# 10XGenomics/rust-pseudoaligner

Measured on AMD Instinct MI355X. Metric: reads/sec pseudoaligned (whole node) on synthetic 150bp reads, higher is better.
Workload: dtype u64; 1 GPU; config3: ~202k-transcript synthetic GENCODE-scale index (K=24), error-free 150bp reads; read_len=150, k=24, transcripts=201914, kmers=103866252, index_bytes=7185579820

## Files before the change

### rust-pseudoaligner_amd/csrc/count_sort.hip

```cpp
#include <hip/hip_runtime.h>

#include <algorithm>

#include "kernels.hpp"
#include "pa_common.hpp"

namespace pa {
namespace {

constexpr uint32_t NO_KEY = 0xFFFFFFFFu;
#ifndef PA_MAX_BINS
#define PA_MAX_BINS 256
#endif
constexpr uint32_t MAX_BINS = PA_MAX_BINS;
constexpr uint64_t PA_COUNT_DIRECT_MAX_READS = 1u << 16;
constexpr uint32_t BIN_SLOTS = 1u << PA_KEY_BIN_SHIFT;
constexpr uint32_t CS_BLOCK = 1024;

struct KeyTops {
    const unsigned long long* top;
    uint64_t cap;
    const unsigned long long* extra_top;
    uint64_t extra_cap;
};
__device__ __forceinline__ uint64_t stream_len(const KeyTops k, uint64_t unused = 0) {
    (void)unused;
    unsigned long long t = *k.top, x = k.extra_top ? *k.extra_top : 0ull;
    if (t > k.cap) t = k.cap;
    if (x > k.extra_cap) x = k.extra_cap;
    return t + x;
}

constexpr uint32_t PT_BLOCK = 512, PT_PER = 16, PT_TILE = PT_BLOCK * PT_PER;

__device__ __forceinline__ uint64_t main_len(const KeyTops k) { const unsigned long long t = *k.top; return t < k.cap ? t : k.cap; }
__device__ __forceinline__ uint64_t extra_len(const KeyTops k) {
    const unsigned long long x = k.extra_top ? *k.extra_top : 0ull;
    return x < k.extra_cap ? x : k.extra_cap;
}
__device__ __forceinline__ uint32_t tiles_of(uint64_t n) { return (uint32_t)((n + PT_TILE - 1) / PT_TILE); }

__global__ __launch_bounds__(PT_BLOCK) void pa_keys_part_kernel(const uint32_t* __restrict__ keys, const KeyTops keys_top, uint32_t pass, uint32_t nbins,
                                                                uint32_t tcap, uint16_t* __restrict__ sorted, uint32_t* __restrict__ run_off) {
    __shared__ uint32_t cnt[MAX_BINS], lbase[MAX_BINS + 1];
    __shared__ __attribute__((aligned(16))) uint16_t stage[PT_TILE];
    const uint64_t m = main_len(keys_top);
    const uint64_t seg0 = pass ? m : 0, len = pass ? extra_len(keys_top) : m;
    const uint32_t tile0 = pass ? tiles_of(m) : 0u, ntiles = tiles_of(len);
    for (uint32_t t = blockIdx.x; t < ntiles; t += gridDim.x) {
        for (uint32_t b = threadIdx.x; b < nbins; b += PT_BLOCK) cnt[b] = 0;
        __syncthreads();
        const uint64_t t0 = (uint64_t)t * PT_TILE;
        uint32_t k[PT_PER], pos[PT_PER];
        const uint4* src = reinterpret_cast<const uint4*>(keys + seg0 + t0) + threadIdx.x;
#pragma unroll
        for (uint32_t j = 0; j < PT_PER / 4; ++j) {
            const uint64_t i = t0 + 4ull * (j * PT_BLOCK + threadIdx.x);
            const uint4 v = i < len ? src[j * PT_BLOCK] : uint4{NO_KEY, NO_KEY, NO_KEY, NO_KEY};
            k[4 * j] = v.x; k[4 * j + 1] = v.y; k[4 * j + 2] = v.z; k[4 * j + 3] = v.w;
        }
#pragma unroll
        for (uint32_t j = 0; j < PT_PER; ++j) pos[j] = k[j] != NO_KEY ? atomicAdd(&cnt[k[j] >> PA_KEY_BIN_SHIFT], 1u) : 0u;
        __syncthreads();
        for (uint32_t b = threadIdx.x; b <= nbins; b += PT_BLOCK) {
            uint32_t s = 0;
            for (uint32_t j = 0; j < b; ++j) s += cnt[j];
            lbase[b] = s;
            run_off[(uint64_t)b * tcap + tile0 + t] = s;
        }
        __syncthreads();
#pragma unroll
        for (uint32_t j = 0; j < PT_PER; ++j)
            if (k[j] != NO_KEY) stage[lbase[k[j] >> PA_KEY_BIN_SHIFT] + pos[j]] = (uint16_t)(k[j] & (BIN_SLOTS - 1));
        __syncthreads();
        uint4* dst = reinterpret_cast<uint4*>(sorted + (uint64_t)(tile0 + t) * PT_TILE);
        const uint32_t n8 = (lbase[nbins] + 7) / 8;
        for (uint32_t i = threadIdx.x; i < n8; i += PT_BLOCK) dst[i] = reinterpret_cast<const uint4*>(stage)[i];
        __syncthreads();
    }
}

constexpr uint32_t CG_LANES = 16, CG_DEPTH = 8;
__global__ __launch_bounds__(CS_BLOCK) void pa_keys_count_kernel(const uint16_t* __restrict__ src, const uint32_t* __restrict__ run_off, uint32_t tcap,
                                                                 const KeyTops keys_top, uint32_t parts, unsigned long long* __restrict__ counts,
                                                                 uint64_t counts_len) {
    extern __shared__ uint32_t tab[];
    const uint32_t bin = blockIdx.x / parts, part = blockIdx.x % parts;
    const uint64_t slot0 = (uint64_t)bin << PA_KEY_BIN_SHIFT;
    const uint32_t nslots = (uint32_t)(counts_len - slot0 < BIN_SLOTS ? counts_len - slot0 : BIN_SLOTS);
    for (uint32_t i = threadIdx.x; i < nslots; i += CS_BLOCK) tab[i] = 0;
    __syncthreads();
    const uint32_t ntiles = tiles_of(main_len(keys_top)) + tiles_of(extra_len(keys_top));
    const uint32_t ta = (uint32_t)((uint64_t)ntiles * part / parts), tb = (uint32_t)((uint64_t)ntiles * (part + 1) / parts);
    const uint32_t gl = threadIdx.x % CG_LANES, group = threadIdx.x / CG_LANES;
    const uint4* q = reinterpret_cast<const uint4*>(src);
    for (uint32_t t = ta + group; t < tb; t += CS_BLOCK / CG_LANES) {
        const uint64_t base = (uint64_t)t * PT_TILE;
        const uint64_t a = base + run_off[(uint64_t)bin * tcap + t], b = base + run_off[(uint64_t)(bin + 1) * tcap + t];
        const uint64_t a8 = (a + 7) & ~7ull, b8 = b & ~7ull;
        if (a8 >= b8) {
            for (uint64_t i = a + gl; i < b; i += CG_LANES) atomicAdd(&tab[src[i]], 1u);
            continue;
        }
        const uint32_t head = a + gl < a8 ? src[a + gl] : 0xFFFFu, tail = b8 + gl < b ? src[b8 + gl] : 0xFFFFu;
        for (uint64_t o0 = a8 / 8; o0 < b8 / 8; o0 += (uint64_t)CG_DEPTH * CG_LANES) {
            uint4 v[CG_DEPTH];
            bool in[CG_DEPTH];
#pragma unroll
            for (uint32_t j = 0; j < CG_DEPTH; ++j) {
                const uint64_t o = o0 + (uint64_t)j * CG_LANES + gl;
                in[j] = o < b8 / 8;
                v[j] = in[j] ? q[o] : uint4{0u, 0u, 0u, 0u};
            }
#pragma unroll
            for (uint32_t j = 0; j < CG_DEPTH; ++j)
                if (in[j]) {
                    atomicAdd(&tab[v[j].x & 0xFFFFu], 1u); atomicAdd(&tab[v[j].x >> 16], 1u);
                    atomicAdd(&tab[v[j].y & 0xFFFFu], 1u); atomicAdd(&tab[v[j].y >> 16], 1u);
                    atomicAdd(&tab[v[j].z & 0xFFFFu], 1u); atomicAdd(&tab[v[j].z >> 16], 1u);
                    atomicAdd(&tab[v[j].w & 0xFFFFu], 1u); atomicAdd(&tab[v[j].w >> 16], 1u);
                }
        }
        if (head != 0xFFFFu) atomicAdd(&tab[head], 1u);
        if (tail != 0xFFFFu) atomicAdd(&tab[tail], 1u);
    }
    __syncthreads();
    for (uint32_t i = threadIdx.x; i < nslots; i += CS_BLOCK) {
        const uint32_t c = tab[i];
        if (c) atomicAdd(counts + slot0 + i, (unsigned long long)c);
    }
}

__global__ __launch_bounds__(CS_BLOCK) void pa_keys_count_raw_kernel(const uint32_t* __restrict__ src, const KeyTops keys_top, unsigned long long* __restrict__ counts,
                                                                     uint64_t counts_len) {
    extern __shared__ uint32_t tab[];
    for (uint32_t i = threadIdx.x; i < counts_len; i += CS_BLOCK) tab[i] = 0;
    __syncthreads();
    const uint64_t n4 = stream_len(keys_top) / 4;
    const uint64_t a = n4 * blockIdx.x / gridDim.x, b = n4 * (blockIdx.x + 1) / gridDim.x;
    const uint4* q = reinterpret_cast<const uint4*>(src);
    for (uint64_t i = a + threadIdx.x; i < b; i += CS_BLOCK) {
        const uint4 v = q[i];
        if (v.x != NO_KEY) atomicAdd(&tab[v.x], 1u);
        if (v.y != NO_KEY) atomicAdd(&tab[v.y], 1u);
        if (v.z != NO_KEY) atomicAdd(&tab[v.z], 1u);
        if (v.w != NO_KEY) atomicAdd(&tab[v.w], 1u);
    }
    __syncthreads();
    for (uint32_t i = threadIdx.x; i < counts_len; i += CS_BLOCK) {
        const uint32_t c = tab[i];
        if (c) atomicAdd(counts + i, (unsigned long long)c);
    }
}

__global__ __launch_bounds__(256) void pa_keys_count_direct_kernel(const uint32_t* __restrict__ keys, const KeyTops keys_top, unsigned long long* __restrict__ counts) {
    const uint64_t n = stream_len(keys_top);
    for (uint64_t i = (uint64_t)blockIdx.x * blockDim.x + threadIdx.x; i < n; i += (uint64_t)gridDim.x * blockDim.x) {
        const uint32_t k = keys[i];
        if (k != NO_KEY) atomicAdd(counts + k, 1ull);
    }
}


}
uint64_t key_stream_capacity(uint64_t n_reads, uint32_t nwaves) {
    return (n_reads / PA_KEY_CHUNK + nwaves + 2) * PA_KEY_CHUNK;
}

static uint64_t nbins_of(uint64_t counts_len) { return (counts_len + BIN_SLOTS - 1) >> PA_KEY_BIN_SHIFT; }

static bool count_direct(uint64_t nbins, uint64_t n_reads) { return nbins > MAX_BINS || (nbins > 1 && n_reads <= PA_COUNT_DIRECT_MAX_READS); }

bool count_keys_partitioned(uint64_t counts_len, uint64_t n_reads) {
    const uint64_t nbins = nbins_of(counts_len);
    return nbins > 1 && !count_direct(nbins, n_reads);
}

static uint32_t tile_capacity(uint64_t keys_cap, uint64_t extra_cap) {
    return (uint32_t)((keys_cap + PT_TILE - 1) / PT_TILE + (extra_cap + PT_TILE - 1) / PT_TILE);
}

void count_keys_scratch(uint64_t counts_len, uint64_t n_reads, uint64_t keys_cap, uint64_t extra_cap, size_t* sorted_bytes, size_t* ctl_bytes) {
    *sorted_bytes = *ctl_bytes = 0;
    if (!count_keys_partitioned(counts_len, n_reads)) return;
    const uint64_t tcap = tile_capacity(keys_cap, extra_cap);
    *sorted_bytes = tcap * PT_TILE * sizeof(uint16_t);
    *ctl_bytes = (nbins_of(counts_len) + 1) * tcap * sizeof(uint32_t);
}

int launch_count_keys(const uint32_t* keys, const unsigned long long* keys_top_ptr, uint64_t keys_cap, const unsigned long long* extra_top, uint64_t extra_cap,
                      uint32_t* sorted, uint32_t* ctl, unsigned long long* counts, uint64_t counts_len, int num_cus, hipStream_t stream, uint64_t n_reads,
                      uint32_t pass) {
    if (counts_len == 0) return 0;
    const KeyTops keys_top{keys_top_ptr, keys_cap, extra_top, extra_cap};
    const uint64_t nbins = nbins_of(counts_len);
    const uint32_t cus = num_cus > 0 ? (uint32_t)num_cus : 256u;
    const bool partitioned = count_keys_partitioned(counts_len, n_reads);
    if (pass == 0) {
        if (!partitioned) return 0;
        const uint32_t tcap = tile_capacity(keys_cap, extra_cap);
        const uint32_t G = std::max<uint32_t>(1u, std::min<uint32_t>(cus * 4, (uint32_t)((keys_cap + PT_TILE - 1) / PT_TILE)));
        hipLaunchKernelGGL(pa_keys_part_kernel, dim3(G), dim3(PT_BLOCK), 0, stream, keys, keys_top, 0u, (uint32_t)nbins, tcap, reinterpret_cast<uint16_t*>(sorted), ctl);
        return (int)hipGetLastError();
    }
    const size_t lds = (size_t)(counts_len < BIN_SLOTS ? counts_len : BIN_SLOTS) * 4;
    if (lds > 48 * 1024) {
        hipError_t e = hipFuncSetAttribute(reinterpret_cast<const void*>(&pa_keys_count_kernel), hipFuncAttributeMaxDynamicSharedMemorySize, (int)lds);
        if (e == hipSuccess) e = hipFuncSetAttribute(reinterpret_cast<const void*>(&pa_keys_count_raw_kernel), hipFuncAttributeMaxDynamicSharedMemorySize, (int)lds);
        if (e != hipSuccess) return (int)e;
    }
    if (count_direct(nbins, n_reads)) {
        const uint32_t blocks = (uint32_t)std::min<uint64_t>((uint64_t)cus * 8, (keys_cap + extra_cap + 255) / 256 + 1);
        hipLaunchKernelGGL(pa_keys_count_direct_kernel, dim3(blocks), dim3(256), 0, stream, keys, keys_top, counts);
        return (int)hipGetLastError();
    }
    if (nbins == 1) {
        hipLaunchKernelGGL(pa_keys_count_raw_kernel, dim3(cus), dim3(CS_BLOCK), lds, stream, keys, keys_top, counts, counts_len);
        return (int)hipGetLastError();
    }
    const uint32_t tcap = tile_capacity(keys_cap, extra_cap);
    const uint32_t G1 = std::max<uint32_t>(1u, std::min<uint32_t>(cus * 4, (uint32_t)((extra_cap + PT_TILE - 1) / PT_TILE)));
    hipLaunchKernelGGL(pa_keys_part_kernel, dim3(G1), dim3(PT_BLOCK), 0, stream, keys, keys_top, 1u, (uint32_t)nbins, tcap, reinterpret_cast<uint16_t*>(sorted), ctl);
    uint32_t parts = std::max<uint32_t>(1u, (uint32_t)(cus / nbins));
    parts = std::max<uint32_t>(1u, (uint32_t)knob_int("PA_COUNT_PARTS", (int)parts));
    hipLaunchKernelGGL(pa_keys_count_kernel, dim3((uint32_t)nbins * parts), dim3(CS_BLOCK), lds, stream, reinterpret_cast<const uint16_t*>(sorted), (const uint32_t*)ctl, tcap,
                       keys_top, parts, counts, counts_len);
    return (int)hipGetLastError();
}

}
```

### rust-pseudoaligner_amd/csrc/resolve.hip

```cpp
#include <hip/hip_runtime.h>

#include "kernel_utils.hpp"
#include "kernels.hpp"
#include "lane_steps.hpp"

namespace pa {
namespace {

constexpr uint32_t NO_KEY = 0xFFFFFFFFu;
typedef uint32_t u32x4 __attribute__((ext_vector_type(4)));

constexpr uint32_t RV_PER = 4;

__global__ __launch_bounds__(256) void pa_resolve_kernel(const MapParams p, uint64_t defer_cap, uint64_t keys_cap) {
    __shared__ unsigned long long s_novel;
    if (threadIdx.x == 0) s_novel = 0;
    __syncthreads();
    const unsigned long long top = *p.defer_top;
    const uint64_t n = top < defer_cap ? top : defer_cap;
    const uint32_t lane = lane_id();
    const bool counting = p.keys != nullptr;
    uint32_t* keys_b = nullptr;
    if (counting) { const unsigned long long kt = *p.keys_top; keys_b = p.keys + (kt < keys_cap ? kt : keys_cap); }
    unsigned long long a_cur = 0, a_end = 0;
    uint32_t my_novel = 0;
    const uint64_t wave0 = ((uint64_t)blockIdx.x * blockDim.x + threadIdx.x) & ~63ull, nwave_lanes = (uint64_t)gridDim.x * blockDim.x;
    for (uint64_t i0 = wave0 * RV_PER; i0 < n; i0 += nwave_lanes * RV_PER) {
        u32x4 e0[RV_PER], e1[RV_PER];
        bool in[RV_PER], live[RV_PER];
        uint64_t idx[RV_PER];
#pragma unroll
        for (uint32_t j = 0; j < RV_PER; ++j) {
            idx[j] = i0 + 64ull * j + lane;
            in[j] = idx[j] < n;
            e0[j] = in[j] ? reinterpret_cast<const u32x4*>(p.defer)[2 * idx[j]] : u32x4{NO_KEY, 0u, 0u, 0u};
        }
#pragma unroll
        for (uint32_t j = 0; j < RV_PER; ++j) {
            live[j] = e0[j].x != NO_KEY;
            e1[j] = live[j] ? reinterpret_cast<const u32x4*>(p.defer)[2 * idx[j] + 1] : u32x4{0u, 0u, 0u, 0u};
        }
        uint32_t colour[RV_PER], want[RV_PER];
        uint32_t wsum = 0;
#pragma unroll
        for (uint32_t j = 0; j < RV_PER; ++j) {
            colour[j] = NO_CLASS;
            const uint32_t count = e0[j].w & 0x3FFFFFFFu;
            if (live[j] && (e0[j].w & PA_DEFER_WINDOW)) {
                uint32_t b1 = e1[j].x, m1 = e1[j].y, b2 = e1[j].z, m2 = e1[j].w;
                window_canon(b1, m1, b2, m2);
                colour[j] = window_class(p.ix, b1, m1, b2, m2);
            } else if (live[j]) {
                colour[j] = class_of_list(p.arena + e1[j].x, count, p.ix, p.class_table, p.class_table_size);
            }
            want[j] = (live[j] && (e0[j].w & PA_DEFER_WINDOW) && colour[j] == NO_CLASS) ? count : 0u;
            wsum += want[j];
        }
        const uint32_t incl = wave_incl_scan(wsum);
        const uint32_t total = (uint32_t)__builtin_amdgcn_readlane((int)incl, 63);
        if (total && a_cur + total > a_end) {
            const unsigned long long take = total > PA_ARENA_CHUNK ? total : PA_ARENA_CHUNK;
            unsigned long long base = 0;
            if (lane == 0) base = atomicAdd(p.arena_top, take);
            a_cur = ((unsigned long long)(uint32_t)__builtin_amdgcn_readfirstlane((int)(base >> 32)) << 32) | (uint32_t)__builtin_amdgcn_readfirstlane((int)base);
            a_end = a_cur + take;
        }
        unsigned long long my_off = a_cur + (incl - wsum);
        a_cur += total;
#pragma unroll
        for (uint32_t j = 0; j < RV_PER; ++j) {
            const uint32_t rid = e0[j].x, cov = e0[j].y, mm = e0[j].z, count = e0[j].w & 0x3FFFFFFFu;
            const bool window = live[j] && (e0[j].w & PA_DEFER_WINDOW);
            bool listed = live[j] && colour[j] == NO_CLASS;
            uint32_t arena_off = e1[j].x;
            if (window) {
                uint32_t class_off = PA_CLASS_REF | colour[j];
                if (want[j]) {
                    class_off = (uint32_t)my_off;
                    arena_off = (uint32_t)my_off;
                    if (my_off + count > p.arena_cap) { atomicOr(p.status, PA_STATUS_ARENA_FULL); listed = false; }
                    else {
                        uint32_t* dst = p.arena + my_off;
                        uint32_t k = 0;
                        for (uint32_t t = e1[j].y; t; t &= t - 1) dst[k++] = e1[j].x + (uint32_t)(__ffs((int)t) - 1);
                        for (uint32_t t = e1[j].w; t; t &= t - 1) dst[k++] = e1[j].z + (uint32_t)(__ffs((int)t) - 1);
                    }
                    my_off += count;
                }
                reinterpret_cast<u32x4*>(p.results)[rid] = u32x4{cov, mm | PA_MAPPED_BIT, class_off, count};
            }
            if (live[j] && p.colour_out) p.colour_out[rid] = colour[j];
            if (live[j] && colour[j] == NO_CLASS) ++my_novel;
            if (counting && in[j]) keys_b[idx[j]] = (live[j] && colour[j] != NO_CLASS) ? colour[j] : NO_KEY;
            if (p.novel_list) {
                const uint64_t m = __ballot(listed);
                if (m) {
                    const uint32_t first = (uint32_t)(__ffsll((unsigned long long)m) - 1);
                    unsigned long long nb = 0;
                    if (lane == first) nb = atomicAdd(p.novel_ctr, (unsigned long long)__popcll(m));
                    nb = ((unsigned long long)(uint32_t)__builtin_amdgcn_readlane((int)(nb >> 32), (int)first) << 32) | (uint32_t)__builtin_amdgcn_readlane((int)nb, (int)first);
                    if (listed) {
                        const unsigned long long at = nb + __builtin_amdgcn_mbcnt_hi((uint32_t)(m >> 32), __builtin_amdgcn_mbcnt_lo((uint32_t)m, 0u));
                        if (at < p.novel_cap) {
                            p.novel_list[2 * at] = arena_off;
                            p.novel_list[2 * at + 1] = count;
                        } else atomicOr(p.novel_status, PA_NOVEL_LIST_FULL);
                    }
                }
            }
        }
    }
    if (counting) {
        if (my_novel) atomicAdd(&s_novel, (unsigned long long)my_novel);
        __syncthreads();
        if (threadIdx.x == 0 && s_novel) atomicAdd(p.counts + p.ix.num_classes, s_novel);
    }
}

}

uint64_t defer_capacity(uint64_t n_reads, uint32_t nwaves) {
    return (n_reads / PA_DEFER_CHUNK + nwaves + 2) * PA_DEFER_CHUNK;
}

int launch_resolve(const MapParams& p, uint64_t defer_cap, uint64_t keys_cap, int num_cus, hipStream_t stream) {
    const uint32_t cus = num_cus > 0 ? (uint32_t)num_cus : 256u;
    hipLaunchKernelGGL(pa_resolve_kernel, dim3(cus * 4), dim3(256), 0, stream, p, defer_cap, keys_cap);
    return (int)hipGetLastError();
}

}
```

Baseline: 13.15 billion reads/s.

## Allocate resolve arena per block with exact-size atomics and rebalance grids

The resolve kernel stops having each wave grab oversized arena chunks. Each block now sums its waves' needs in shared memory and makes one exact-size atomicAdd per pass, with double-buffered shared slots and two __syncthreads per iteration. Items per lane drop from 4 to 2 and the grid grows from 4 to 16 blocks per CU, which should improve latency hiding and balance. The partition kernel grid in count_sort is also halved. The cost is block-wide barriers on every pass; the intended gain is less wasted arena space and more parallelism.

After: 13.29 billion reads/s, median of 6. 1.0% higher.

```diff
diff --git a/rust-pseudoaligner_amd/csrc/count_sort.hip b/rust-pseudoaligner_amd/csrc/count_sort.hip
--- a/rust-pseudoaligner_amd/csrc/count_sort.hip
+++ b/rust-pseudoaligner_amd/csrc/count_sort.hip
@@ -199,7 +199,7 @@
     if (pass == 0) {
         if (!partitioned) return 0;
         const uint32_t tcap = tile_capacity(keys_cap, extra_cap);
-        const uint32_t G = std::max<uint32_t>(1u, std::min<uint32_t>(cus * 4, (uint32_t)((keys_cap + PT_TILE - 1) / PT_TILE)));
+        const uint32_t G = std::max<uint32_t>(1u, std::min<uint32_t>(cus * 2, (uint32_t)((keys_cap + PT_TILE - 1) / PT_TILE)));
         hipLaunchKernelGGL(pa_keys_part_kernel, dim3(G), dim3(PT_BLOCK), 0, stream, keys, keys_top, 0u, (uint32_t)nbins, tcap, reinterpret_cast<uint16_t*>(sorted), ctl);
         return (int)hipGetLastError();
     }
diff --git a/rust-pseudoaligner_amd/csrc/resolve.hip b/rust-pseudoaligner_amd/csrc/resolve.hip
--- a/rust-pseudoaligner_amd/csrc/resolve.hip
+++ b/rust-pseudoaligner_amd/csrc/resolve.hip
@@ -10,9 +10,11 @@
 constexpr uint32_t NO_KEY = 0xFFFFFFFFu;
 typedef uint32_t u32x4 __attribute__((ext_vector_type(4)));
 
-constexpr uint32_t RV_PER = 4;
+constexpr uint32_t RV_PER = 2;
+constexpr uint32_t RV_BLOCK = 256, RV_WAVES = RV_BLOCK / 64;
+constexpr uint64_t RV_PASS = (uint64_t)RV_BLOCK * RV_PER;
 
-__global__ __launch_bounds__(256) void pa_resolve_kernel(const MapParams p, uint64_t defer_cap, uint64_t keys_cap) {
+__global__ __launch_bounds__(RV_BLOCK) void pa_resolve_kernel(const MapParams p, uint64_t defer_cap, uint64_t keys_cap) {
     __shared__ unsigned long long s_novel;
     if (threadIdx.x == 0) s_novel = 0;
     __syncthreads();
@@ -22,10 +24,12 @@
     const bool counting = p.keys != nullptr;
     uint32_t* keys_b = nullptr;
     if (counting) { const unsigned long long kt = *p.keys_top; keys_b = p.keys + (kt < keys_cap ? kt : keys_cap); }
-    unsigned long long a_cur = 0, a_end = 0;
-    uint32_t my_novel = 0;
-    const uint64_t wave0 = ((uint64_t)blockIdx.x * blockDim.x + threadIdx.x) & ~63ull, nwave_lanes = (uint64_t)gridDim.x * blockDim.x;
-    for (uint64_t i0 = wave0 * RV_PER; i0 < n; i0 += nwave_lanes * RV_PER) {
+    __shared__ uint32_t s_tot[2][RV_WAVES];
+    __shared__ unsigned long long s_base[2];
+    uint32_t my_novel = 0, par = 0;
+    const uint32_t wave = threadIdx.x >> 6;
+    for (uint64_t g0 = (uint64_t)blockIdx.x * RV_PASS; g0 < n; g0 += (uint64_t)gridDim.x * RV_PASS, par ^= 1u) {
+        const uint64_t i0 = g0 + (uint64_t)wave * 64 * RV_PER;
         u32x4 e0[RV_PER], e1[RV_PER];
         bool in[RV_PER], live[RV_PER];
         uint64_t idx[RV_PER];
@@ -58,15 +62,22 @@
         }
         const uint32_t incl = wave_incl_scan(wsum);
         const uint32_t total = (uint32_t)__builtin_amdgcn_readlane((int)incl, 63);
-        if (total && a_cur + total > a_end) {
-            const unsigned long long take = total > PA_ARENA_CHUNK ? total : PA_ARENA_CHUNK;
-            unsigned long long base = 0;
-            if (lane == 0) base = atomicAdd(p.arena_top, take);
-            a_cur = ((unsigned long long)(uint32_t)__builtin_amdgcn_readfirstlane((int)(base >> 32)) << 32) | (uint32_t)__builtin_amdgcn_readfirstlane((int)base);
-            a_end = a_cur + take;
+        if (lane == 0) s_tot[par][wave] = total;
+        __syncthreads();
+        if (threadIdx.x == 0) {
+            uint32_t sum = 0;
+#pragma unroll
+            for (uint32_t w = 0; w < RV_WAVES; ++w) sum += s_tot[par][w];
+            if (sum) s_base[par] = atomicAdd(p.arena_top, (unsigned long long)sum);
         }
-        unsigned long long my_off = a_cur + (incl - wsum);
-        a_cur += total;
+        __syncthreads();
+        unsigned long long my_off = 0;
+        if (total) {
+            uint32_t before = incl - wsum;
+#pragma unroll
+            for (uint32_t w = 0; w < RV_WAVES; ++w) before += w < wave ? s_tot[par][w] : 0u;
+            my_off = s_base[par] + before;
+        }
 #pragma unroll
         for (uint32_t j = 0; j < RV_PER; ++j) {
             const uint32_t rid = e0[j].x, cov = e0[j].y, mm = e0[j].z, count = e0[j].w & 0x3FFFFFFFu;
@@ -125,7 +136,7 @@
 
 int launch_resolve(const MapParams& p, uint64_t defer_cap, uint64_t keys_cap, int num_cus, hipStream_t stream) {
     const uint32_t cus = num_cus > 0 ? (uint32_t)num_cus : 256u;
-    hipLaunchKernelGGL(pa_resolve_kernel, dim3(cus * 4), dim3(256), 0, stream, p, defer_cap, keys_cap);
+    hipLaunchKernelGGL(pa_resolve_kernel, dim3(cus * 16), dim3(RV_BLOCK), 0, stream, p, defer_cap, keys_cap);
     return (int)hipGetLastError();
 }
 
```
